# bloomberg/blazingmq

Measured on AMD Instinct MI355X. Metric: device-resident CRC32C GiB/s over batched payloads, 1/2/4/8 MI355X, higher is better.
Workload: dtype u32; 1 GPU; 64k_x_64KiB: 65,536 msgs x 64 KiB per GPU (configs[2], HBM-bound headline); payload_bytes_total=4294967296, seg_bytes=auto, whole_messages=False, parallelism=dp1 (sharded batch, no collective)

## Files before the change

blazingmq_amd/csrc/bmqcrc_host.cpp:

```cpp
#include <hip/hip_runtime.h>
#include <stdint.h>
#include <stdio.h>
#include <stdlib.h>
#include <string.h>

#include <algorithm>
#include <atomic>
#include <condition_variable>
#include <initializer_list>
#include <map>
#include <memory>
#include <mutex>
#include <string>
#include <thread>
#include <utility>
#include <vector>

#include "../../include/bmqcrc.h"
#include "../../include/bmqcrc_protocol.h"
#include "bmqcrc_internal.h"

namespace bmqcrc {
uint32_t cpu_crc32c(const void* data, uint32_t length, uint32_t crc);
uint32_t cpu_combine(uint32_t crcA, uint32_t crcB, uint64_t lenB);
// ... 51 lines not shown
        fresh = true;
        if (p) {
            (void)hipFree(p);
            p = nullptr;
            bytes = 0;
        }
        want = std::max<uint64_t>(want, 256);
        HIP_TRY(hipMalloc(&p, want));
        bytes = want;
        return 0;
    }
    ~DevBuf()
    {
        if (p) {
            (void)hipFree(p);
        }
    }
};

struct PackScratch {
    DevBuf off, first, out, bsum, copy_bsum, ctr;
    uint64_t n = 0;
    bool any = false;
    int ensure(uint64_t n_msgs, int ctr_words, bool need_out)
    {
        int rc;
        if ((rc = ctr.ensure(8 * (ctr_words + kCopyCtrWords))) ||
            (rc = bsum.ensure(8ull * 2 * kPackBlocks)) || (rc = off.ensure(8 * n_msgs))) {
            return rc;
        }
        return need_out ? out.ensure(4 * n_msgs) : 0;
    }
};

struct UnpackScratch {
    DevBuf off, len, exp, out, ctr;
    uint64_t n = 0;
    bool any = false;
    int ensure(uint64_t msg_cap, bool need_out, int ctr_words = kSlotCtrWords)
    {
        const uint64_t slots = std::max<uint64_t>(msg_cap, 1);
        int rc;
        if ((rc = ctr.ensure(8 * ctr_words)) || (rc = off.ensure(8 * slots)) ||
            (rc = len.ensure(4 * slots)) || (rc = exp.ensure(4 * slots))) {
            return rc;
        }
        return need_out ? out.ensure(4 * slots) : 0;
    }
};

struct Workspace {
    std::mutex mu;
    DevBuf seg_first, block_sum, seginfo, firstk, gdesc, grec, bhist, plan_sync;
    uint32_t plan_epoch = 0;
    uint64_t map_wait_ticks = 10000;

    DevBuf arena, offsets, lengths, seeds, out;
    DevBuf expected, vcount, vidx, vblock, buf_crc, first_buf;
    std::vector<std::pair<hipEvent_t, hipEvent_t>> timing, spare;
    uint32_t* hint_host = nullptr;
    uint32_t* hint_dev = nullptr;
    uint32_t last_kernels = 0, last_spec = 0, last_seg = 0, last_map = 0;
    uint32_t last_off_bits = 64, last_off_shift = 0;
    uint32_t void_seen = 0, pair_left = 0;
    DevBuf copy_first, copy_bsum, copy_ctr;
    uint64_t copy_n = 0;
    bool copy_any = false;
    PackScratch pack, rec;
    uint64_t pack_events = 0;
    UnpackScratch unp, runp;
    DevBuf unp_first, unp_bad;
    DevBuf runp_pre, runp_roff, runp_rlen, runp_rflags, runp_bsum;
    UnpackScratch sap;
    DevBuf sap_first, sap_bad, sap_dst, sap_jrn, sap_rec, sap_hdr, sap_pay, sap_meta, sap_bsum;
    DevBuf sap_copy_first, sap_copy_bsum;
    uint32_t sap_lease = 0;
    uint64_t sap_seq = 0;
    UnpackScratch spk;
    DevBuf spk_dst, spk_rec, spk_hdr, spk_type, spk_bsum, spk_copy_first, spk_copy_bsum;
    uint64_t spk_events = 0;
    UnpackScratch ppk;
    DevBuf ppk_dst, ppk_meta, ppk_bsum, ppk_copy_first, ppk_copy_bsum;
    uint64_t ppk_events = 0;
    DevBuf jsel_zero, jsel_rec;
    uint64_t jsel_records = 0;
    bool jsel_any = false;
    uint8_t* pin = nullptr;
    hipEvent_t pin_ev[16] = {};
    bool pin_used[16] = {};
    ~Workspace()
    {
        if (hint_host) {
            (void)hipHostFree(hint_host);
        }
        if (pin) {
            (void)hipHostFree(pin);
        }
        for (hipEvent_t e : pin_ev) {
            if (e) {
                (void)hipEventDestroy(e);
            }
        }
        for (auto& v : {timing, spare}) {
            for (auto& e : v) {
                (void)hipEventDestroy(e.first);
                (void)hipEventDestroy(e.second);
// ... 168 lines not shown
}

struct Ctx {
    int dev = 0;
    DeviceState* st = nullptr;
    hipStream_t s = nullptr;
    Workspace* w = nullptr;
};

int open_ctx(int dev, void* user_stream, Ctx* c)
{
    int rc = device_state(dev, &c->st);
    if (rc) {
        return rc;
    }
    HIP_TRY(hipSetDevice(dev));
    c->dev = dev;
    c->s = (hipStream_t)user_stream;
    c->w = workspace(dev, user_stream);
    return 0;
}

struct LockedCtx : Ctx {
    std::unique_lock<std::mutex> lock;
};

int lock_on(int device, void* stream, bool with_state, LockedCtx* c)
{
    int dev, rc;
    if ((rc = resolve_device(device, &dev))) {
        return rc;
    }
    if (with_state) {
        if ((rc = open_ctx(dev, stream, c))) {
            return rc;
        }
    } else {
        c->dev = dev;
        c->s = (hipStream_t)stream;
        c->w = workspace(dev, stream);
    }
    c->lock = std::unique_lock<std::mutex>(c->w->mu);
    return 0;
}

bool spec_eligible(const Ctx& c, uint64_t n, uint32_t blocks_per_cu)
{
    const uint32_t per_cu = (kTuneBits & 2u) ? 1u : (kTuneBits & 8u) ? 2u : blocks_per_cu;
    const uint64_t waves = (uint64_t)(c.st->num_cus > 0 ? c.st->num_cus : 256) * per_cu *
                           kWavesPerBlock;
    return (n + 63) / 64 >= waves;
}

void auto_shape(uint64_t n, uint64_t arena_bytes, int num_cus, uint32_t* seg,
                uint32_t* blocks_per_cu)
{
    const uint64_t cus = (uint64_t)(num_cus > 0 ? num_cus : 256);
    const uint64_t wave_segs = (uint64_t)kWavesPerBlock * kWaveLanes;
    const bool large = n > 0 && arena_bytes / n >= kDefaultSegBytes;
    if (large && arena_bytes / (4 * kDefaultSegBytes) >= cus * wave_segs) {
        *blocks_per_cu = 1;
        if (*seg == 0) {
            *seg = 4 * kDefaultSegBytes;
        }
        return;
    }
    *blocks_per_cu = 2;
    if (*seg == 0) {
        const uint64_t slots = cus * 2 * wave_segs;
        if (large && arena_bytes / kDefaultSegBytes >= slots) {
            *seg = kDefaultSegBytes;
            return;
        }
        *seg = 256;
        for (uint32_t s : {2048u, 1024u, 512u}) {
            if (arena_bytes / s >= 2 * slots) {
                *seg = s;
                break;
            }
        }
    }
}

uint64_t max_length(const uint32_t* lengths, uint64_t n)
{
    uint32_t m = 0;
    for (uint64_t i = 0; i < n; ++i) {
        m = std::max(m, lengths[i]);
    }
    return m;
}

uint64_t min_length(const uint32_t* lengths, uint64_t n)
{
    uint32_t m = n ? UINT32_MAX : 0u;
    for (uint64_t i = 0; i < n; ++i) {
        m = std::min(m, lengths[i]);
    }
    return m;
}

int run_batch(Ctx& c, uint32_t flags, uint32_t seg, const void* arena, uint64_t arena_bytes,
              const uint64_t* offsets, const uint32_t* lengths, const uint32_t* seeds,
              uint32_t* out, uint64_t n, uint64_t host_max_len = UINT64_MAX,
              uint64_t host_min_len = 0, uint32_t off_shift = 0)
{
    Workspace* w = c.w;
    BatchArgs a;
    memset(&a, 0, sizeof(a));
    a.n = n;
    a.off32 = (flags & BMQCRC_F_OFFSETS32) ? 1u : 0u;
    a.off_shift = a.off32 ? off_shift : 0u;
    auto_shape(n, arena_bytes, c.st->num_cus, &seg, &a.blocks_per_cu);
    a.seg_bytes = seg;
    a.tune = kTuneBits;
    int rc;
    if (flags & BMQCRC_F_WHOLE_MESSAGES) {
        a.whole = 1;
        a.max_segs = n;
    } else if ((rc = plan_ws(w, c.s, n, arena_bytes, seg, &a, *c.st, a.off32 != 0))) {
        return rc;
    } else if (!(kTuneBits & 16u) && !(flags & BMQCRC_F_PLAN)) {
        const uint32_t hint = __atomic_load_n(w->hint_host, __ATOMIC_RELAXED);
        const uint32_t shape = hint & 0xffu, hint_u = hint >> 8;
        if (shape == kHintClosed || shape == kHintIdentity) {
            a.map_planned = 0;
        }
        if (shape == kHintIdentity && spec_eligible(c, n, a.blocks_per_cu)) {
            a.spec = 1;
        } else if (shape == kHintClosed && hint_u >= 2u && hint_u <= 64u && 64u % hint_u == 0u &&
                   (uint64_t)n * hint_u <= 0xFFFFFF00ull) {
            a.spec = hint_u;
        }
    }
    hipStreamCaptureStatus cap = hipStreamCaptureStatusNone;
    const bool capturing = hipStreamIsCapturing(c.s, &cap) == hipSuccess &&
                           cap == hipStreamCaptureStatusActive;
    if (!(kTuneBits & (16u | 4096u)) && !capturing && !a.whole && !a.spec && a.map_planned &&
        w->hint_host &&
        (__atomic_load_n(w->hint_host, __ATOMIC_RELAXED) & 0xffu) != kHintRagged &&
        !(host_max_len != UINT64_MAX && host_max_len > a.seg_bytes &&
          (host_min_len == 0 || (host_min_len - 1) / a.seg_bytes != (host_max_len - 1) / a.seg_bytes))) {
        a.map_planned = 0;
    }
    if ((kTuneBits & 2048u) && !a.whole && (flags & BMQCRC_F_PLAN) &&
        spec_eligible(c, n, a.blocks_per_cu)) {
        a.spec = 1;
    } else if (!a.whole && host_max_len <= a.seg_bytes && !(flags & BMQCRC_F_PLAN)) {
        a.spec = 1;
    } else if (!a.whole && host_min_len > 0 && host_max_len != UINT64_MAX &&
               !(flags & BMQCRC_F_PLAN)) {
        const uint64_t u = (host_max_len - 1) / a.seg_bytes + 1;
        if ((host_min_len - 1) / a.seg_bytes + 1 == u && u >= 2 && u <= 64 && 64 % u == 0 &&
            (uint64_t)n * u <= 0xFFFFFF00ull) {
            a.spec = (uint32_t)u;
        }
    }
    if (!a.whole && !a.spec && a.map_planned && w->hint_host && w->map_wait_ticks != 0) {
        const uint32_t voided = __atomic_load_n(w->hint_host + 1, __ATOMIC_RELAXED);
        if (voided != w->void_seen) {
            w->void_seen = voided;
            w->pair_left = kPairAfterVoid;
        }
        if (w->pair_left) {
            a.pair = 1;
            --w->pair_left;
        }
    }
    if (!a.whole && !a.spec && a.map_planned) {
        if (capturing) {
            a.plan_epoch = 0;
        }
    }
    a.arena = (const uint8_t*)arena;
    a.offsets = offsets;
    a.lengths = lengths;
    a.seeds = seeds;
    a.out = out;
    void* ev0 = nullptr;
    void* ev1 = nullptr;
    if (flags & BMQCRC_F_TIME_KERNEL) {
        std::pair<hipEvent_t, hipEvent_t> ev;
        if (!w->spare.empty()) {
            ev = w->spare.back();
            w->spare.pop_back();
        } else {
            HIP_TRY(hipEventCreate(&ev.first));
            HIP_TRY(hipEventCreate(&ev.second));
        }
        w->timing.push_back(ev);
        ev0 = (void*)ev.first;
        ev1 = (void*)ev.second;
    }
    if (bmqcrc_launch_batch(&a, (void*)c.s, c.st->num_cus, ev0, ev1) != 0) {
        return fail(BMQCRC_EIO, std::string("kernel launch failed: ") +
                                    hipGetErrorString(hipGetLastError()));
    }
    w->last_spec = a.whole ? 1u : a.spec;
    w->last_seg = a.seg_bytes;
    w->last_kernels = n == 0                 ? 0u
                      : (a.whole || a.spec)  ? 1u
                      : !a.map_planned       ? 2u
                      : single_pass_planner(a) ? 2u
                                             : 3u;
    w->last_map = n != 0 && !a.whole && !a.spec && a.map_planned ? 1u : 0u;
    w->last_off_bits = a.off32 ? 32u : 64u;
    w->last_off_shift = a.off_shift;
    return 0;
// ... 2944 lines not shown
```

blazingmq_amd/csrc/bmqcrc_internal.h:

```cpp
#pragma once
#include <stddef.h>
#include <stdint.h>

namespace bmqcrc {

constexpr int kLine = 128;
constexpr int kWaveLanes = 64;
constexpr int kWavesPerBlock = 4;
constexpr int kSlots = 2;
constexpr int kSlotBytes = kWaveLanes * kLine;
constexpr int kLdsBytes = kWavesPerBlock * kSlots * kSlotBytes;
constexpr int kTabBytes = 8 * 256 * 4;
constexpr int kXbBytes = 4 * 256 * 4;
constexpr uint32_t kDefaultSegBytes = 16384;
constexpr int kPlanBlock = 1024;
constexpr int kPlanMaxBlocks = 256;
constexpr int kSyncFlags = 16;

constexpr int kBuckets = 16;

#ifndef BMQCRC_TUNE_BITS
#define BMQCRC_TUNE_BITS 0u
#endif
constexpr uint32_t kTuneBits = BMQCRC_TUNE_BITS;
constexpr uint32_t kRightAlignLines = 1u;

struct BatchArgs {
    const uint8_t* arena;
    const uint64_t* offsets;
    const uint32_t* lengths;
    const uint32_t* seeds;
    uint32_t* out;
    uint32_t* seg_first;
    uint32_t* block_sum;
    uint32_t* seginfo;
    uint32_t* firstk;
    unsigned long long* gdesc;
    uint32_t* grec;
    uint32_t* bhist;
    uint64_t n;
    uint64_t max_segs;
    uint64_t per_msg;
    uint32_t seg_bytes;
    uint32_t nblocks;
    uint32_t whole;
    uint32_t blocks_per_cu;
    uint32_t tune;
    uint32_t map_planned;
    uint32_t* shape_hint;
    uint32_t spec;
    unsigned long long* plan_sync;
    uint32_t plan_epoch;
    uint32_t off32;
    uint64_t map_wait_ticks;
    uint32_t class_desc;
    uint32_t pair;
    uint32_t spread;
    uint32_t off_shift;
};

static_assert(sizeof(BatchArgs) == 200 && offsetof(BatchArgs, plan_epoch) == 168 &&
                  offsetof(BatchArgs, off32) == 172 && offsetof(BatchArgs, map_wait_ticks) == 176 &&
                  offsetof(BatchArgs, spread) == 192 && offsetof(BatchArgs, off_shift) == 196,
              "BatchArgs: kernel argument offsets are fixed");

constexpr uint32_t kPairAfterVoid = 16;

constexpr uint64_t kClassDescGroupsPerWave = 24;

constexpr uint32_t kPlanV = 4;
constexpr uint32_t kSegLast = 0x80000000u;

inline bool single_pass_planner(const BatchArgs& a)
{
    return !(a.tune & 128u) && !a.pair;
}

constexpr uint32_t kHintUnknown = 0;
constexpr uint32_t kHintClosed = 1;
constexpr uint32_t kHintRagged = 2;
constexpr uint32_t kHintIdentity = 3;

constexpr int kCopyWaves = 4;
constexpr uint32_t kCopyChunkPieces = 4096;
constexpr uint32_t kCopyChunkBytes = 16 * kCopyChunkPieces;
constexpr int kCopyPlanThreads = 1024;
constexpr uint32_t kCopyPlanBlocks = 256;
constexpr int kCopyCtrRefused = 0;
constexpr int kCopyCtrLowestInv = 1;
constexpr int kCopyCtrOverflow = 2;
constexpr int kCopyCtrWords = 4;

// ... 439 lines not shown
```

blazingmq_amd/csrc/crc32c_kernels.hip:

```cpp
#include <hip/hip_runtime.h>
#include <stdint.h>

#include <algorithm>

#include "bmqcrc_internal.h"
#include "crc32c_consts.h"
#include "crc32c_diag.h"

namespace bmqcrc {

typedef __attribute__((address_space(3))) uint8_t lds_u8;
typedef __attribute__((address_space(3))) uint32_t lds_u32;
typedef uint32_t u32x4 __attribute__((ext_vector_type(4)));
typedef __attribute__((address_space(3))) const u32x4 lds_cu4;
typedef __attribute__((address_space(3))) u32x4 lds_u4;
typedef uint64_t u64x2 __attribute__((ext_vector_type(2)));
typedef uint32_t u32x4e __attribute__((ext_vector_type(4), aligned(4)));
typedef uint64_t u64x2e __attribute__((ext_vector_type(2), aligned(8)));

__constant__ uint32_t c_x2col[31][32] = BMQCRC_X2COL;
__constant__ uint32_t c_xneg8[136] = BMQCRC_XNEG8;
__constant__ uint32_t c_xbytes[4][256] = BMQCRC_XBYTES;
__constant__ uint32_t c_ty[8][256] = BMQCRC_TY;
__constant__ uint32_t c_rtab11[6144] = BMQCRC_RTAB11;
// ... 714 lines not shown
    const uint32_t lane = (uint32_t)(threadIdx.x & 63);
    const uint32_t key = valid ? r.msg : 0xffffffffu;
    const uint32_t prev = (uint32_t)__shfl_up((int)key, 1);
    const bool head = lane == 0 || prev != key || (key & kSegLast);
    const uint64_t heads = __ballot(head);
    const uint64_t upto = lane == 63 ? ~0ull : ((2ull << lane) - 1ull);
    const uint32_t h = 63u - (uint32_t)__builtin_clzll(heads & upto);
    SegRef o;
    o.msg = key & ~kSegLast;
    o.k = (key & kSegLast) ? kKFromLength : (h == 0 ? r.k : 0u) + (lane - h);
    return o;
}

template <bool O32>
__device__ __forceinline__ uint64_t raw_offset(const BatchArgs& a, uint64_t i)
{
    if constexpr (O32) {
        return ((const uint32_t*)a.offsets)[i];
    } else {
        return a.offsets[i];
    }
}

template <bool O32>
__device__ __forceinline__ uint64_t wide_offset(const BatchArgs& a, uint64_t raw)
{
    if constexpr (O32) {
        return raw << a.off_shift;
    } else {
        return raw;
    }
}

template <bool O32>
__device__ __forceinline__ uint64_t msg_offset(const BatchArgs& a, uint64_t i)
{
    return wide_offset<O32>(a, raw_offset<O32>(a, i));
}

template <bool O32>
__device__ __forceinline__ SegDesc fetch_desc(const BatchArgs& a, SegRef r, bool valid)
{
    SegDesc d = {0ull, r.msg, r.k, 0u, 0u};
    if (valid) {
        d.off = raw_offset<O32>(a, r.msg);
        d.len = a.lengths[r.msg];
        d.seed = a.seeds ? a.seeds[r.msg] : 0u;
    }
    return d;
}

constexpr uint32_t kLongListCap = 64;

template <bool NT, bool ONE, int WPB, bool O32>
__global__ __launch_bounds__(WPB * 64, WPB == 4 ? 2 : 1) void k_fold(BatchArgs a)
{
    constexpr uint32_t kThreads = WPB * 64;
    constexpr int kLds = WPB * kSlots * kSlotBytes;
    constexpr bool H11 = WPB == 8;
    constexpr int kTab = H11 ? (int)kTab11Bytes : kTabBytes;
    __shared__ __attribute__((aligned(16))) uint8_t lds[kTab + kLds + (ONE ? 0 : kXbBytes)];
    __shared__ uint32_t claim_ctr, long_n;
    [[maybe_unused]] __shared__ unsigned long long claim2;
    __shared__ uint32_t long_list[kLongListCap];
    __shared__ uint32_t one_prog[WPB];

    const int lane = threadIdx.x & 63;
    const uint32_t wave = __builtin_amdgcn_readfirstlane(threadIdx.x >> 6);
    const uint32_t tab_lds = (uint32_t)(uintptr_t)(lds_u8*)lds;
    const uint32_t wave_lds = tab_lds + kTab + wave * (kSlots * kSlotBytes);
    const uint32_t xb_lds = tab_lds + kTab + kLds;
    auto remainder = [&](const uint32_t (&Rm)[32], bool skip) -> uint32_t {
        if constexpr (H11) {
            return skip ? tail_bytes8<true>(Rm, tab_lds) : tail_bytes8<false>(Rm, tab_lds);
        } else {
            return skip ? tail_bytes8<true, true>(Rm, tab_lds) : tail_bytes8<false, true>(Rm, tab_lds);
        }
    };
    if (threadIdx.x < (uint32_t)WPB) {
        one_prog[threadIdx.x] = 0u;
    }
    if (threadIdx.x == 0) {
        claim_ctr = WPB;
        claim2 = 0ull;
        long_n = 0;
    }

    constexpr int kTw = (kTab / 4) / (int)kThreads, kXw = 1024 / kThreads;
    static_assert(kTw * (int)kThreads * 4 == kTab && kXw * kThreads == 1024, "table fill");
    constexpr bool kEarly = ONE && WPB == 4;
    static_assert(!kEarly || kTab % (1024 * WPB) == 0, "early tables: whole KiB per wave");
    constexpr bool kNoVgprTab = kEarly;
    const uint32_t gfirst = a.spread ? wave * gridDim.x + blockIdx.x : blockIdx.x * WPB + wave;
    const uint32_t sid = gfirst * 64u + (uint32_t)lane;
    const SegDesc spec = fetch_desc<O32>(a, SegRef{sid, 0u}, sid < a.n);
    uint32_t tw[kNoVgprTab ? 1 : kTw];
#pragma unroll
    for (int i = 0; i < (kNoVgprTab ? 0 : kTw); ++i) {
        const uint32_t t = threadIdx.x + (uint32_t)i * kThreads;
        if constexpr (H11) {
            tw[i] = c_rtab11[t];
        } else {
            tw[i] = c_ty[t >> 8][t & 255u];
        }
    }
    uint32_t xw[kXw];
    if (!ONE) {
#pragma unroll
        for (int i = 0; i < kXw; ++i) {
            const uint32_t t = threadIdx.x + (uint32_t)i * kThreads;
            xw[i] = c_xbytes[t >> 8][t & 255u];
        }
    }
    const uint32_t whole = ONE ? 0u : a.whole;
    const uint32_t spec_mode = ONE ? 1u : a.spec;
    const uint32_t spec_u = spec_mode ? spec_mode : 1u;
    PlanWords pw = {0u, 0u, 0u, 0u};
    uint32_t map_void = 0u;
    uint32_t ep = a.plan_epoch;
    if (!whole && !spec_mode) {
        pw = plan_load(a);
        if (a.map_planned && a.plan_sync) {
            ep = launch_epoch(a);
            map_void = (uint32_t)a.plan_sync[2] == ep;
        }
    }
    __shared__ __attribute__((aligned(16))) uint32_t xneg8[136];
    const uint32_t xn = (!kNoVgprTab && threadIdx.x < 136u) ? c_xneg8[threadIdx.x] : 0u;
    [[maybe_unused]] const uint32_t g0 = blockIdx.x * WPB + wave;
    FOLD_STAMP(0)
#pragma unroll
    for (int i = 0; i < (kNoVgprTab ? 0 : kTw); ++i) {
        const uint32_t t = threadIdx.x + (uint32_t)i * kThreads;
        *(lds_u32*)(uintptr_t)(tab_lds + 4u * t) = tw[i];
    }
    if (!kNoVgprTab && threadIdx.x < 136u) {
        xneg8[threadIdx.x] = xn;
    }
    auto early_tables = [&]() {
        if constexpr (kEarly) {
            constexpr int kKib = kTab / 1024 / WPB;
            const uint64_t src = H11 ? (uint64_t)(uintptr_t)&c_rtab11[0]
                                     : (uint64_t)(uintptr_t)&c_ty[0][0];
            dma_copy_kib<kKib>(tab_lds + 1024u * kKib * wave, src + 1024u * kKib * wave);
            if (wave == 0 && lane < 34) {
                dma_copy_kib<1>((uint32_t)(uintptr_t)xneg8, (uint64_t)(uintptr_t)&c_xneg8[0]);
            }
        }
    };
    auto early_barrier = [&](bool wait) {
        if constexpr (kEarly) {
            if (wait) {
                asm volatile("s_waitcnt vmcnt(0)" ::: "memory");
            }
            __builtin_amdgcn_s_barrier();
        }
    };
    if (!ONE) {
#pragma unroll
        for (int i = 0; i < kXw; ++i) {
            const uint32_t t = threadIdx.x + (uint32_t)i * kThreads;
            *(lds_u32*)(uintptr_t)(xb_lds + 4u * t) = xw[i];
        }
    }

    __shared__ PlanLds pl;
    PlanTotals pt = {(uint32_t)a.n * spec_u, spec_u == 1u ? 1u : 0u, spec_u == 1u ? 0u : spec_u,
                     0u};
    if (!whole && !spec_mode) {
        pt = plan_reduce(a, &pl, pw);
    } else {
        __syncthreads();
    }
    const uint32_t wholef = whole | pt.overflow;
    const uint32_t hint_identity = pt.identity && !pt.overflow;
    const uint32_t hint_uni = pt.uni;
    if (pt.overflow) {
        pt.identity = 1u;
        pt.uni = 0u;
        pt.total = (uint32_t)a.n;
    }
    const uint32_t total = pt.total;
    const uint32_t identity = pt.identity;
    const uint32_t uni = pt.uni;
    const uint32_t sorted =
        (wholef || !a.map_planned || identity || uni || total > a.max_segs || map_void) ? 0u : 1u;
    const uint32_t ngroups = (total + 63u) / 64u;
    const uint32_t SEG = a.seg_bytes;
    const uint64_t arena = (uint64_t)(uintptr_t)a.arena;
    if (a.shape_hint && blockIdx.x == 0 && threadIdx.x == 0 && !whole && !spec_mode) {
        __hip_atomic_store(a.shape_hint,
                           hint_identity ? kHintIdentity
                           : (hint_uni && !pt.overflow && 64u % hint_uni == 0u)
                               ? (kHintClosed | (hint_uni << 8))
                           : (hint_uni || pt.overflow) ? kHintClosed
                                                  : kHintRagged,
                           __ATOMIC_RELAXED, __HIP_MEMORY_SCOPE_SYSTEM);
        if (map_void) {
            __hip_atomic_store(a.shape_hint + 1, ep, __ATOMIC_RELAXED,
                               __HIP_MEMORY_SCOPE_SYSTEM);
        }
    }

    FOLD_STAMP(1)
    const uint32_t rd_off = (uint32_t)lane * 128u + (((uint32_t)lane >> 1) & 7u) * 16u;
    const uint64_t zero = (uint64_t)(uintptr_t)g_zero_line + 16u * ((uint32_t)lane & 7u);

    const uint32_t nbk = gridDim.x;
    auto gid = [&](uint32_t k) {
        if (a.spread) {
            return k * nbk + blockIdx.x;
        }
        const uint32_t r = k / (uint32_t)WPB;
        const uint32_t b = (!ONE && (r & 1u)) ? nbk - 1u - blockIdx.x : blockIdx.x;
        return (b + nbk * r) * (uint32_t)WPB + k % (uint32_t)WPB;
    };
    auto claim_issue = [&]() {
        unsigned long long k = 0;
        if (lane == 0) {
            k = atomicAdd(&claim_ctr, 1u);
        }
        return k;
    };
    auto claim_take = [&](unsigned long long k) {
        return gid((uint32_t)__builtin_amdgcn_readfirstlane((int)(uint32_t)k));
    };
    auto claim = [&]() { return claim_take(claim_issue()); };
    const uint32_t seg_shift = (SEG & (SEG - 1u)) == 0 ? (uint32_t)__builtin_ctz(SEG) : 0u;

    struct Group {
        uint64_t pbase[8];
        uint32_t plo[8], pcnt[8];
        uint64_t E, L0, mend;
        uint32_t msg, k, nseg, nl, R, r0, sl, jE, eE, c0, hskip;
        bool valid, first, lo_part, hi_part;
        bool whole_lines;
    };
    auto setup_lane = [&](bool valid, uint32_t msg, uint32_t k, uint32_t nseg, uint64_t off,
                          uint32_t len, uint32_t seed, Group& G) {
        G.valid = valid;
        G.msg = msg;
        G.k = k;
        G.nseg = valid ? nseg : 0u;
        const uint64_t mstart = arena + off;
        G.mend = mstart + len;
        const SegGeom geo = seg_geom(mstart, len, G.k, G.nseg, SEG);
        G.E = geo.E;
        G.L0 = geo.L0;
        G.first = G.valid && G.k == 0;
        G.nl = G.valid ? geo.nl : 0u;
        G.R = max(wave_max(G.nl), 1u);
        G.hskip = 0u;
        if (G.R == 1u) {
            const uint32_t sl0 = G.valid ? (uint32_t)(geo.S - geo.L0) : 128u;
            G.hskip = __ballot(sl0 < 64u) == 0 ? 8u : 0u;
        }
        G.r0 = G.R - G.nl;
        G.sl = G.valid ? (uint32_t)(geo.S - G.L0) : 0u;
        const uint64_t el = G.valid ? G.E - G.L0 : 0u;
        G.lo_part = (G.sl & 15u) != 0;
        G.hi_part = (el & 15u) != 0;
        G.jE = (uint32_t)(el >> 7);
        G.eE = (uint32_t)(el & 127u);
        G.c0 = ~seed;
        G.whole_lines = __ballot(G.valid && (((geo.S | geo.E) & 127u) != 0)) == 0;
        const uint32_t gS = G.sl >> 4;
        const uint32_t gE = (uint32_t)((el + 15u) >> 4);
        const uint32_t plo_l = 8u * G.r0 + gS;
        const uint32_t pcnt_l = G.valid ? gE - gS : 0u;
        const uint64_t pb_l = G.L0 - ((uint64_t)G.r0 << 7);
        const uint32_t ls = (uint32_t)lane;
        const uint32_t kq = ls >> 3;
        *(lds_u4*)(uintptr_t)(wave_lds + 16u * ((ls & 7u) * 8u + (kq ^ (ls & 7u)))) =
            u32x4{(uint32_t)pb_l, (uint32_t)(pb_l >> 32), plo_l, pcnt_l};
        __builtin_amdgcn_wave_barrier();
#pragma unroll
        for (int i = 0; i < 8; ++i) {
            const u32x4 v = *(lds_cu4*)(uintptr_t)(wave_lds + 16u * (kq * 8u + ((uint32_t)i ^ kq)));
            const uint32_t pp = ((uint32_t)lane & 7u) ^ ((4u * i + ((uint32_t)lane >> 4)) & 7u);
            G.pbase[i] = (((uint64_t)v.y << 32) | v.x) + 16u * pp;
            G.plo[i] = v.z - pp;
            G.pcnt[i] = v.w;
        }
    };
    auto segments = [&](uint32_t len) {
        return len ? (seg_shift ? ((len - 1u) >> seg_shift) : (len - 1u) / SEG) + 1u : 0u;
    };
    bool long_seen = false;
    auto setup = [&](const SegDesc& d, uint32_t gg, Group& G) {
        const uint32_t seg = gg * 64u + (uint32_t)lane;
        bool valid = seg < total;
        uint32_t nseg = !valid ? 0u : (wholef ? 1u : segments(d.len));
        if (spec_mode) {
            const bool ok = spec_u == 1u ? nseg <= 1u : nseg == spec_u;
            if constexpr (ONE) {
                long_seen |= __ballot(valid && !ok) != 0;
            } else if (__ballot(valid && !ok) != 0 && lane == 0) {
                const uint32_t at = atomicAdd(&long_n, 1u);
                if (at < kLongListCap) {
                    long_list[at] = gg;
                }
            }
            valid = valid && ok;
            nseg = spec_u;
        }
        if (ONE) {
            setup_lane(valid, d.msg, 0u, 1u, wide_offset<O32>(a, d.off), d.len, d.seed, G);
        } else {
            setup_lane(valid, d.msg, d.k == kKFromLength ? nseg - 1u : d.k, nseg,
                       wide_offset<O32>(a, d.off), d.len, d.seed, G);
        }
    };
    auto issue_first_rounds = [&](const Group& G) {
        if (!NT || (G.R <= 2u && !G.whole_lines)) {
            dma_round<false>(wave_lds, G.pbase, G.plo, G.pcnt, zero, 0);
            if (G.R > 1) {
                dma_round<false>(wave_lds + kSlotBytes, G.pbase, G.plo, G.pcnt, zero, 1);
            }
            return;
        }
        dma_round<true>(wave_lds, G.pbase, G.plo, G.pcnt, zero, 0);
        if (G.R > 1) {
            dma_round<true>(wave_lds + kSlotBytes, G.pbase, G.plo, G.pcnt, zero, 1);
        }
    };

    auto fold_rounds = [&](const Group& G, uint32_t (&Rm)[32]) {
        uint32_t q[32], p[32];
        const uint32_t R = G.R;
        auto load_line = [&](uint32_t r, uint32_t slot, uint32_t (&m)[32]) {
            const uint32_t j = r - G.r0;
            const bool fx_lo = G.lo_part && j == 0u;
            const bool fx_hi = G.hi_part && j == G.jE;
            const bool fx_sd = G.first && (j == 0u || (j == 1u && G.sl > 124u));
            if (__ballot(fx_lo || fx_hi || fx_sd)) {
                if (fx_lo || fx_hi || fx_sd) {
                    line_fixup(slot, rd_off, fx_lo, G.sl, fx_hi, G.eE, fx_sd,
                               (int)(G.sl - 128u * j), G.c0);
                }
            }
#pragma unroll
            for (int kk = 0; kk < 8; ++kk) {
                const u32x4 v = *(lds_cu4*)(uintptr_t)(slot + (rd_off ^ (16u * kk)));
                m[4 * kk + 0] = v.x;
                m[4 * kk + 1] = v.y;
                m[4 * kk + 2] = v.z;
                m[4 * kk + 3] = v.w;
            }
        };
        for (uint32_t r = 0; r + 1 < R; ++r) {
// ... 1 lines not shown
            asm volatile("s_waitcnt vmcnt(0)" ::: "memory");
            uint32_t m[32];
            load_line(r, slot, m);
            if (r + 2 < R) {
                dma_round<NT>(slot, G.pbase, G.plo, G.pcnt, zero, r + 2);
            }
            if (r == 0) {
                first_round(q, p, m);
            } else {
                fold_round(q, p, m);
            }
        }
        const uint32_t slot = wave_lds + ((R - 1u) & 1u) * kSlotBytes;
        if (R == 1) {
            asm volatile("s_waitcnt vmcnt(0)" ::: "memory");
            load_line(0u, slot, Rm);
            return;
        }
        uint32_t H[32];
        tail_taps(q, p, H);
        asm volatile("s_waitcnt vmcnt(0)" ::: "memory");
        uint32_t m[32];
        load_line(R - 1u, slot, m);
#pragma unroll
        for (int d = 0; d < 32; ++d) {
            Rm[d] = m[d] ^ H[d];
        }
    };

    auto contribution = [&](const Group& C, uint32_t crc) {
        uint32_t contrib = 0;
        const uint32_t padE = C.valid ? (uint32_t)(C.L0 + ((uint64_t)C.nl << 7) - C.E) : 0u;
        if (__ballot(padE != 0) == 0) {
            contrib = C.valid ? crc : 0u;
        } else if (C.valid) {
            contrib = gmul(crc, xneg8[padE]);
        }
        if (ONE) {
            contrib = mul_xpow(contrib, C.valid ? mersenne31(8ull * (C.mend - C.E)) : 0u);
        } else {
            contrib = mul_xbytes(contrib, C.valid ? (uint32_t)(C.mend - C.E) : 0u, xb_lds);
        }
        if (C.first) {
            contrib ^= 0xffffffffu;
        }
        return contrib;
    };
    struct Pending {
        uint32_t msg, val, mode;
    };
    auto commit = [&](const Pending& P) {
        if (P.mode == 1u) {
            a.out[P.msg] = P.val;
        } else if (P.mode == 2u) {
            atomicXor(&a.out[P.msg], P.val);
        }
    };
    auto finish = [&](const Group& C, uint32_t crc) -> Pending {
        Pending P = {C.msg, 0u, 0u};
        if (ONE) {
            uint32_t contrib = C.valid ? crc : 0u;
            const uint32_t padE = C.valid ? (uint32_t)(C.L0 + ((uint64_t)C.nl << 7) - C.E) : 0u;
            if (__ballot(padE != 0) != 0 && C.valid) {
                contrib = gmul(crc, xneg8[padE]);
            }
            P.val = contrib ^ 0xffffffffu;
            P.mode = C.valid ? 1u : 0u;
            return P;
        }
        uint32_t contrib = contribution(C, crc);
        if (__ballot(C.valid && C.nseg != 1u) == 0) {
            P.val = contrib;
            P.mode = C.valid ? 1u : 0u;
            return P;
        }
        const uint32_t key = C.valid ? C.msg : 0xffffffffu;
        const uint32_t pkey = (uint32_t)__shfl_up((int)key, 1);
        const bool head = lane == 0 || pkey != key;
        const uint64_t heads = __ballot(head);
        const uint64_t upto = (lane == 63) ? ~0ull : ((2ull << lane) - 1ull);
        const uint64_t later = heads & ~upto;
        const uint32_t rend = later ? (uint32_t)__builtin_ctzll(later) : 64u;
#pragma unroll
        for (int o = 1; o < 64; o <<= 1) {
            const uint32_t ov = (uint32_t)__shfl_down((int)contrib, o);
            if ((uint32_t)lane + (uint32_t)o < rend) {
                contrib ^= ov;
            }
        }
        P.val = contrib;
        if (C.valid && head) {
            P.mode = (C.k == 0 && rend - (uint32_t)lane == C.nseg) ? 1u : 2u;
        }
        return P;
    };

    auto second_pass = [&](uint32_t nlong) {
        bool any = false;
        const uint32_t mpg = 64u / spec_u;
        const bool listed = nlong <= kLongListCap;
        for (uint32_t j = wave;; j += WPB) {
            const uint32_t gg = ONE ? gfirst + (j / (uint32_t)WPB) * nbk * (uint32_t)WPB
                                : listed ? (j < nlong ? long_list[j] : ngroups) : gid(j);
            if (gg >= ngroups) {
                break;
            }
            const uint64_t i = (uint64_t)gg * mpg + (uint32_t)lane;
            const bool mine = (uint32_t)lane < mpg && i < a.n;
            const uint32_t len = mine ? a.lengths[i] : 0u;
            const uint32_t ns = segments(len);
            uint64_t todo = __ballot(mine && (spec_u == 1u ? ns > 1u : ns != spec_u));
            any = any || todo != 0;
            for (; todo; todo &= todo - 1ull) {
                const uint32_t msg = (uint32_t)((uint64_t)gg * mpg + __builtin_ctzll(todo));
                const uint64_t off = msg_offset<O32>(a, msg);
                const uint32_t mlen = a.lengths[msg];
                const uint32_t seed = a.seeds ? a.seeds[msg] : 0u;
                const uint32_t nseg = segments(mlen);
                uint32_t acc = mlen ? 0u : seed;
                for (uint32_t c = 0; 64u * c < nseg; ++c) {
                    const uint32_t k = 64u * c + (uint32_t)lane;
                    Group H;
                    setup_lane(k < nseg, msg, k, nseg, off, mlen, seed, H);
                    issue_first_rounds(H);
                    uint32_t Rm[32];
                    fold_rounds(H, Rm);
                    uint32_t x = contribution(H, remainder(Rm, false));
#pragma unroll
                    for (int o = 32; o > 0; o >>= 1) {
                        x ^= (uint32_t)__shfl_xor((int)x, o);
                    }
                    acc ^= x;
                }
                if (lane == 0) {
                    a.out[msg] = acc;
                }
            }
        }
        if (any && lane == 0 && a.shape_hint) {
            __hip_atomic_store(a.shape_hint, kHintRagged, __ATOMIC_RELAXED,
                               __HIP_MEMORY_SCOPE_SYSTEM);
        }
    };

    Group G;
    SegDesc nxt = {0ull, 0u, 0u, 0u, 0u};
    SegRef ref2 = {0u, 0u};
    if constexpr (ONE) {
        const uint32_t stride = nbk * (uint32_t)WPB;
        uint32_t g = gfirst;
        if (g < ngroups) {
            const uint32_t s0 = g * 64u + (uint32_t)lane;
            SegRef r0 = {0u, 0u};
            if (!identity) {
                r0 = map_segment(a, &pl, s0, s0 < total, identity, uni, sorted, ep);
                if (sorted) {
                    r0 = resolve_sorted(r0, s0 < total);
                }
            }
            const SegDesc d0 = identity ? spec : fetch_desc<O32>(a, r0, s0 < total);
            const uint32_t s1 = (g + stride) * 64u + (uint32_t)lane;
            const bool v1 = g + stride < ngroups && s1 < total;
            SegRef r1 = map_segment(a, &pl, s1, v1, identity, uni, sorted, ep);
            if (sorted) {
                r1 = resolve_sorted(r1, v1);
            }
            if constexpr (!kNoVgprTab) {
// ... 33 lines not shown
                        __builtin_amdgcn_s_setprio(1);
                    }
                    ++it;
                }
            }
            uint32_t Rm[32];
            fold_rounds(G, Rm);
            if (meet) {
                early_barrier(false);
                meet = false;
            }
            if (first) {
                FOLD_STAMP(3)
                first = false;
            }
            if (g + stride >= ngroups) {
                FOLD_STAMP(4)
            }
            const Group C = G;
            if (g + stride < ngroups) {
                setup(nxt, g + stride, G);
                const uint32_t s2 = (g + 2u * stride) * 64u + (uint32_t)lane;
                const bool v2 = g + 2u * stride < ngroups && s2 < total;
                nxt = fetch_desc<O32>(a, sorted ? resolve_sorted(ref2, v2) : ref2, v2);
                const uint32_t s3 = (g + 3u * stride) * 64u + (uint32_t)lane;
                ref2 = map_segment(a, &pl, s3, g + 3u * stride < ngroups && s3 < total, identity,
                                   uni, sorted, ep);
                issue_first_rounds(G);
            }
            commit(pend);
            pend = finish(C, remainder(Rm, C.hskip != 0u));
        }
        commit(pend);
    } else {
    uint32_t g = gid(wave), g1 = ngroups, g2 = ngroups;
    if (g < ngroups) {
        g1 = claim();
        g2 = g1 < ngroups ? claim() : ngroups;
        const uint32_t s0 = g * 64u + (uint32_t)lane;
        SegRef r0 = {0u, 0u};
        if (!identity) {
            r0 = map_segment(a, &pl, s0, s0 < total, identity, uni, sorted, ep);
            if (sorted) {
                r0 = resolve_sorted(r0, s0 < total);
            }
        }
        const SegDesc d0 = identity ? spec : fetch_desc<O32>(a, r0, s0 < total);
        const uint32_t s1 = g1 * 64u + (uint32_t)lane;
        const bool v1 = g1 < ngroups && s1 < total;
        SegRef r1 = map_segment(a, &pl, s1, v1, identity, uni, sorted, ep);
        if (sorted) {
            r1 = resolve_sorted(r1, v1);
        }
        nxt = fetch_desc<O32>(a, r1, v1);
        const uint32_t s2 = g2 * 64u + (uint32_t)lane;
        ref2 = map_segment(a, &pl, s2, g2 < ngroups && s2 < total, identity, uni, sorted, ep);
        setup(d0, g, G);
        issue_first_rounds(G);
        FOLD_STAMP(2)
    }
    bool first_group = true;
    Pending pend = {0u, 0u, 0u};
    while (g < ngroups) {
        const bool more = g1 < ngroups && g2 < ngroups;
        const unsigned long long k3 = more ? claim_issue() : 0ull;
        uint32_t Rm[32];
        fold_rounds(G, Rm);
        if (first_group) {
            FOLD_STAMP(3)
            first_group = false;
        }
        if (g1 >= ngroups) {
            FOLD_STAMP(4)
        }
        const Group C = G;
        uint32_t g3 = ngroups;
        if (g1 < ngroups) {
            setup(nxt, g1, G);
            const uint32_t s2 = g2 * 64u + (uint32_t)lane;
            const bool v2 = g2 < ngroups && s2 < total;
            nxt = fetch_desc<O32>(a, sorted ? resolve_sorted(ref2, v2) : ref2, v2);
            g3 = more ? claim_take(k3) : ngroups;
            const uint32_t s3 = g3 * 64u + (uint32_t)lane;
            ref2 = map_segment(a, &pl, s3, g3 < ngroups && s3 < total, identity, uni, sorted, ep);
            issue_first_rounds(G);
        }
        commit(pend);
        pend = finish(C, remainder(Rm, C.hskip != 0u));
        g = g1;
        g1 = g2;
        g2 = g3;
    }
    commit(pend);
    }
    FOLD_STAMP(5)
    if constexpr (ONE) {
        if (long_seen) {
            second_pass(0u);
        }
    } else if (spec_mode) {
        __syncthreads();
        const uint32_t nlong = long_n;
        if (nlong) {
            second_pass(nlong);
        }
    }
    FOLD_STAMP(6)
}

__device__ __forceinline__ uint32_t size_class(uint32_t nl)
{
    nl |= 1u;
    const uint32_t b = 31u - __clz(nl);
    const uint32_t c = b ? 2u * b + ((nl >> (b - 1u)) & 1u) : 0u;
    return c < kBuckets - 1 ? c : kBuckets - 1;
}

__device__ __forceinline__ uint32_t msg_segments(const BatchArgs& a, uint64_t off, uint32_t len,
                                                 uint32_t seg_shift, uint32_t* c_last)
{
// ... 544 lines not shown

}

using namespace bmqcrc;

template <bool O32>
static int launch_batch(const BatchArgs* a, void* stream, int num_cus, void* ev_start,
                        void* ev_stop)
{
    hipStream_t s = (hipStream_t)stream;
    if (a->n == 0) {
        return 0;
    }
    if (!a->whole && !a->spec && a->map_planned && a->plan_epoch == 0) {
        hipLaunchKernelGGL(k_epoch_advance, dim3(1), dim3(1), 0, s, a->plan_sync);
    }
    if (!a->whole && !a->spec) {
        const bool single_pass = single_pass_planner(*a);
        if (a->map_planned && single_pass) {
            hipLaunchKernelGGL(O32 ? k_plan_map32 : k_plan_map, dim3(a->nblocks), dim3(kPlanBlock), 0, s, *a);
        } else if (a->map_planned) {
            hipLaunchKernelGGL((k_plan<true, O32>), dim3(a->nblocks), dim3(kPlanBlock), 0, s, *a);
        } else {
            hipLaunchKernelGGL((k_plan<false, O32>), dim3(a->nblocks), dim3(kPlanBlock), 0, s, *a);
        }
        if (a->map_planned && !single_pass) {
            hipLaunchKernelGGL(k_plan_sort<O32>, dim3(a->nblocks), dim3(kPlanBlock), 0, s, *a);
        }
    }
    const uint64_t max_groups = (a->max_segs + 63) / 64;
    const uint32_t per_cu = (a->tune & 2u) ? 1u : (a->tune & 8u) ? 2u : a->blocks_per_cu;
    const uint64_t cus = (uint64_t)(num_cus > 0 ? num_cus : 256);
    const bool wide = per_cu == 2u && !(a->tune & 1024u) && max_groups >= 2u * 8u * cus;
    const uint32_t wpb = wide ? 8u : 4u;
    uint64_t grid = (max_groups + wpb - 1) / wpb;
    const uint64_t cap = wide ? cus : cus * (per_cu ? per_cu : 2u);
    if (grid > cap) {
        grid = cap;
    }
    if (grid < 1) {
        grid = 1;
    }
    if (ev_start) {
        (void)hipEventRecord((hipEvent_t)ev_start, s);
    }
    const bool one = a->spec == 1u && !a->whole && !(a->tune & 64u);
    BatchArgs b = *a;
    b.spread = 0u;
    if (!wide && grid < cus && max_groups > grid) {
        grid = std::min<uint64_t>(max_groups, cus);
        b.spread = 1u;
    }
    const dim3 gd((unsigned)grid), bd(wpb * 64u);
    if (a->tune & 1u) {
        if (wide) {
            hipLaunchKernelGGL((k_fold<false, false, 8, O32>), gd, bd, 0, s, b);
        } else {
            hipLaunchKernelGGL((k_fold<false, false, 4, O32>), gd, bd, 0, s, b);
        }
    } else if (one) {
        if (wide) {
            hipLaunchKernelGGL((k_fold<true, true, 8, O32>), gd, bd, 0, s, b);
        } else {
            hipLaunchKernelGGL((k_fold<true, true, 4, O32>), gd, bd, 0, s, b);
        }
    } else if (wide) {
        hipLaunchKernelGGL((k_fold<true, false, 8, O32>), gd, bd, 0, s, b);
    } else {
        hipLaunchKernelGGL((k_fold<true, false, 4, O32>), gd, bd, 0, s, b);
    }
    if (ev_stop) {
        (void)hipEventRecord((hipEvent_t)ev_stop, s);
    }
    return hipGetLastError() == hipSuccess ? 0 : -5;
}

extern "C" int bmqcrc_launch_batch(const BatchArgs* a, void* stream, int num_cus, void* ev_start,
                                   void* ev_stop)
{
    return a->off32 ? launch_batch<true>(a, stream, num_cus, ev_start, ev_stop)
                    : launch_batch<false>(a, stream, num_cus, ev_start, ev_stop);
}

extern "C" int bmqcrc_plan_map_occupancy(int off32, int* blocks_per_cu)
{
    int per = 0;
    const void* k = off32 ? reinterpret_cast<const void*>(&k_plan_map32)
                          : reinterpret_cast<const void*>(&k_plan_map);
    if (hipOccupancyMaxActiveBlocksPerMultiprocessor(&per, k, kPlanBlock, 0) != hipSuccess) {
        return -5;
    }
    *blocks_per_cu = per;
    return 0;
}

extern "C" int bmqcrc_launch_compare(const uint32_t* got, const uint32_t* expected, uint64_t n,
                                     uint32_t* bad_count, uint32_t* bad_idx, uint32_t bad_cap,
                                     void* stream)
{
    if (n == 0) {
        return 0;
    }
    const uint64_t blocks = std::min<uint64_t>((n + 255) / 256, 4096);
    hipLaunchKernelGGL(k_compare, dim3((unsigned)blocks), dim3(256), 0, (hipStream_t)stream, got,
                       expected, n, bad_count, bad_idx, bad_cap);
    return hipGetLastError() == hipSuccess ? 0 : -5;
}
// ... 51 lines not shown
```

Measured before the change: 6590 GiB/s.

## Add SPEC kernel variant for uniform multi-group messages with arrival counters

```diff
diff --git a/blazingmq_amd/csrc/bmqcrc_host.cpp b/blazingmq_amd/csrc/bmqcrc_host.cpp
--- a/blazingmq_amd/csrc/bmqcrc_host.cpp
+++ b/blazingmq_amd/csrc/bmqcrc_host.cpp
@@ -127,6 +127,8 @@
 struct Workspace {
     std::mutex mu;
     DevBuf seg_first, block_sum, seginfo, firstk, gdesc, grec, bhist, plan_sync;
+    DevBuf arrive;
+    bool arrive_zeroed = false;
     uint32_t plan_epoch = 0;
     uint64_t map_wait_ticks = 10000;
 
@@ -401,6 +403,12 @@
     return (n + 63) / 64 >= waves;
 }
 
+bool spec_uniform(uint64_t u, uint64_t n)
+{
+    return u >= 2 && (u <= 64 ? 64 % u == 0 : u % 64 == 0 && u < (1u << 24)) &&
+           n * u <= 0xFFFFFF00ull;
+}
+
 void auto_shape(uint64_t n, uint64_t arena_bytes, int num_cus, uint32_t* seg,
                 uint32_t* blocks_per_cu)
 {
@@ -477,8 +485,7 @@
         }
         if (shape == kHintIdentity && spec_eligible(c, n, a.blocks_per_cu)) {
             a.spec = 1;
-        } else if (shape == kHintClosed && hint_u >= 2u && hint_u <= 64u && 64u % hint_u == 0u &&
-                   (uint64_t)n * hint_u <= 0xFFFFFF00ull) {
+        } else if (shape == kHintClosed && spec_uniform(hint_u, n)) {
             a.spec = hint_u;
         }
     }
@@ -500,9 +507,23 @@
     } else if (!a.whole && host_min_len > 0 && host_max_len != UINT64_MAX &&
                !(flags & BMQCRC_F_PLAN)) {
         const uint64_t u = (host_max_len - 1) / a.seg_bytes + 1;
-        if ((host_min_len - 1) / a.seg_bytes + 1 == u && u >= 2 && u <= 64 && 64 % u == 0 &&
-            (uint64_t)n * u <= 0xFFFFFF00ull) {
+        if ((host_min_len - 1) / a.seg_bytes + 1 == u && spec_uniform(u, n)) {
             a.spec = (uint32_t)u;
+        }
+    }
+    if (a.spec > 64u) {
+        if ((rc = w->arrive.ensure(8 * n))) {
+            return rc;
+        }
+        w->arrive_zeroed = w->arrive_zeroed && !w->arrive.fresh;
+        if (!w->arrive_zeroed && capturing) {
+            a.spec = 0;
+        } else if (!w->arrive_zeroed) {
+            HIP_TRY(hipMemsetAsync(w->arrive.p, 0, w->arrive.bytes, c.s));
+            w->arrive_zeroed = true;
+        }
+        if (a.spec) {
+            a.arrive = (unsigned long long*)w->arrive.p;
         }
     }
     if (!a.whole && !a.spec && a.map_planned && w->hint_host && w->map_wait_ticks != 0) {
diff --git a/blazingmq_amd/csrc/bmqcrc_internal.h b/blazingmq_amd/csrc/bmqcrc_internal.h
--- a/blazingmq_amd/csrc/bmqcrc_internal.h
+++ b/blazingmq_amd/csrc/bmqcrc_internal.h
@@ -37,7 +37,10 @@
     uint32_t* firstk;
     unsigned long long* gdesc;
     uint32_t* grec;
-    uint32_t* bhist;
+    union {
+        uint32_t* bhist;
+        unsigned long long* arrive;
+    };
     uint64_t n;
     uint64_t max_segs;
     uint64_t per_msg;
diff --git a/blazingmq_amd/csrc/crc32c_kernels.hip b/blazingmq_amd/csrc/crc32c_kernels.hip
--- a/blazingmq_amd/csrc/crc32c_kernels.hip
+++ b/blazingmq_amd/csrc/crc32c_kernels.hip
@@ -790,9 +790,10 @@
 
 constexpr uint32_t kLongListCap = 64;
 
-template <bool NT, bool ONE, int WPB, bool O32>
+template <bool NT, bool ONE, int WPB, bool O32, bool SPEC = false>
 __global__ __launch_bounds__(WPB * 64, WPB == 4 ? 2 : 1) void k_fold(BatchArgs a)
 {
+    static_assert(!(ONE && SPEC), "ONE is a speculative kernel of its own");
     constexpr uint32_t kThreads = WPB * 64;
     constexpr int kLds = WPB * kSlots * kSlotBytes;
     constexpr bool H11 = WPB == 8;
@@ -826,7 +827,7 @@
 
     constexpr int kTw = (kTab / 4) / (int)kThreads, kXw = 1024 / kThreads;
     static_assert(kTw * (int)kThreads * 4 == kTab && kXw * kThreads == 1024, "table fill");
-    constexpr bool kEarly = ONE && WPB == 4;
+    constexpr bool kEarly = (ONE || SPEC) && WPB == 4;
     static_assert(!kEarly || kTab % (1024 * WPB) == 0, "early tables: whole KiB per wave");
     constexpr bool kNoVgprTab = kEarly;
     const uint32_t gfirst = a.spread ? wave * gridDim.x + blockIdx.x : blockIdx.x * WPB + wave;
@@ -843,7 +844,7 @@
         }
     }
     uint32_t xw[kXw];
-    if (!ONE) {
+    if (!ONE && !kEarly) {
 #pragma unroll
         for (int i = 0; i < kXw; ++i) {
             const uint32_t t = threadIdx.x + (uint32_t)i * kThreads;
@@ -853,10 +854,12 @@
     const uint32_t whole = ONE ? 0u : a.whole;
     const uint32_t spec_mode = ONE ? 1u : a.spec;
     const uint32_t spec_u = spec_mode ? spec_mode : 1u;
+    const uint32_t gpm = (SPEC && spec_u > 64u) ? spec_u / 64u : 1u;
+    const bool planned = !SPEC && !whole && !spec_mode;
     PlanWords pw = {0u, 0u, 0u, 0u};
     uint32_t map_void = 0u;
     uint32_t ep = a.plan_epoch;
-    if (!whole && !spec_mode) {
+    if (planned) {
         pw = plan_load(a);
         if (a.map_planned && a.plan_sync) {
             ep = launch_epoch(a);
@@ -881,6 +884,11 @@
             const uint64_t src = H11 ? (uint64_t)(uintptr_t)&c_rtab11[0]
                                      : (uint64_t)(uintptr_t)&c_ty[0][0];
             dma_copy_kib<kKib>(tab_lds + 1024u * kKib * wave, src + 1024u * kKib * wave);
+            if constexpr (!ONE) {
+                static_assert(kXbBytes == 1024 * WPB, "early tables: a KiB of move factors per wave");
+                dma_copy_kib<1>(xb_lds + 1024u * wave,
+                                (uint64_t)(uintptr_t)&c_xbytes[0][0] + 1024u * wave);
+            }
             if (wave == 0 && lane < 34) {
                 dma_copy_kib<1>((uint32_t)(uintptr_t)xneg8, (uint64_t)(uintptr_t)&c_xneg8[0]);
             }
@@ -894,7 +902,7 @@
             __builtin_amdgcn_s_barrier();
         }
     };
-    if (!ONE) {
+    if (!ONE && !kEarly) {
 #pragma unroll
         for (int i = 0; i < kXw; ++i) {
             const uint32_t t = threadIdx.x + (uint32_t)i * kThreads;
@@ -905,7 +913,7 @@
     __shared__ PlanLds pl;
     PlanTotals pt = {(uint32_t)a.n * spec_u, spec_u == 1u ? 1u : 0u, spec_u == 1u ? 0u : spec_u,
                      0u};
-    if (!whole && !spec_mode) {
+    if (planned) {
         pt = plan_reduce(a, &pl, pw);
     } else {
         __syncthreads();
@@ -926,10 +934,12 @@
     const uint32_t ngroups = (total + 63u) / 64u;
     const uint32_t SEG = a.seg_bytes;
     const uint64_t arena = (uint64_t)(uintptr_t)a.arena;
-    if (a.shape_hint && blockIdx.x == 0 && threadIdx.x == 0 && !whole && !spec_mode) {
+    if (a.shape_hint && blockIdx.x == 0 && threadIdx.x == 0 && planned) {
         __hip_atomic_store(a.shape_hint,
                            hint_identity ? kHintIdentity
-                           : (hint_uni && !pt.overflow && 64u % hint_uni == 0u)
+                           : (hint_uni && !pt.overflow &&
+                              (64u % hint_uni == 0u ||
+                               (hint_uni % 64u == 0u && hint_uni < (1u << 24))))
                                ? (kHintClosed | (hint_uni << 8))
                            : (hint_uni || pt.overflow) ? kHintClosed
                                                   : kHintRagged,
@@ -1033,7 +1043,7 @@
             const bool ok = spec_u == 1u ? nseg <= 1u : nseg == spec_u;
             if constexpr (ONE) {
                 long_seen |= __ballot(valid && !ok) != 0;
-            } else if (__ballot(valid && !ok) != 0 && lane == 0) {
+            } else if (__ballot(valid && !ok) != 0 && lane == 0 && gg % gpm == 0u) {
                 const uint32_t at = atomicAdd(&long_n, 1u);
                 if (at < kLongListCap) {
                     long_list[at] = gg;
@@ -1141,8 +1151,18 @@
     auto commit = [&](const Pending& P) {
         if (P.mode == 1u) {
             a.out[P.msg] = P.val;
-        } else if (P.mode == 2u) {
+        } else if (!SPEC && P.mode == 2u) {
             atomicXor(&a.out[P.msg], P.val);
+        } else if (SPEC && P.mode == 3u) {
+            unsigned long long* const word = a.arrive + P.msg;
+            __hip_atomic_fetch_xor(word, (unsigned long long)P.val, __ATOMIC_RELAXED,
+                                   __HIP_MEMORY_SCOPE_AGENT);
+            const unsigned long long before = __hip_atomic_fetch_add(
+                word, 1ull << 32, __ATOMIC_RELAXED, __HIP_MEMORY_SCOPE_AGENT);
+            if ((uint32_t)(before >> 32) + 1u == gpm) {
+                __hip_atomic_store(word, 0ull, __ATOMIC_RELAXED, __HIP_MEMORY_SCOPE_AGENT);
+                a.out[P.msg] = (uint32_t)before;
+            }
         }
     };
     auto finish = [&](const Group& C, uint32_t crc) -> Pending {
@@ -1179,14 +1199,14 @@
         }
         P.val = contrib;
         if (C.valid && head) {
-            P.mode = (C.k == 0 && rend - (uint32_t)lane == C.nseg) ? 1u : 2u;
+            P.mode = (C.k == 0 && rend - (uint32_t)lane == C.nseg) ? 1u : SPEC ? 3u : 2u;
         }
         return P;
     };
 
     auto second_pass = [&](uint32_t nlong) {
         bool any = false;
-        const uint32_t mpg = 64u / spec_u;
+        const uint32_t mpg = gpm > 1u ? 1u : 64u / spec_u;
         const bool listed = nlong <= kLongListCap;
         for (uint32_t j = wave;; j += WPB) {
             const uint32_t gg = ONE ? gfirst + (j / (uint32_t)WPB) * nbk * (uint32_t)WPB
@@ -1194,14 +1214,15 @@
             if (gg >= ngroups) {
                 break;
             }
-            const uint64_t i = (uint64_t)gg * mpg + (uint32_t)lane;
-            const bool mine = (uint32_t)lane < mpg && i < a.n;
+            const uint64_t m0 = (uint64_t)(gg / gpm) * mpg;
+            const uint64_t i = m0 + (uint32_t)lane;
+            const bool mine = (uint32_t)lane < mpg && i < a.n && gg % gpm == 0u;
             const uint32_t len = mine ? a.lengths[i] : 0u;
             const uint32_t ns = segments(len);
             uint64_t todo = __ballot(mine && (spec_u == 1u ? ns > 1u : ns != spec_u));
             any = any || todo != 0;
             for (; todo; todo &= todo - 1ull) {
-                const uint32_t msg = (uint32_t)((uint64_t)gg * mpg + __builtin_ctzll(todo));
+                const uint32_t msg = (uint32_t)(m0 + __builtin_ctzll(todo));
                 const uint64_t off = msg_offset<O32>(a, msg);
                 const uint32_t mlen = a.lengths[msg];
                 const uint32_t seed = a.seeds ? a.seeds[msg] : 0u;
@@ -1341,20 +1362,37 @@
         if (sorted) {
             r1 = resolve_sorted(r1, v1);
         }
-        nxt = fetch_desc<O32>(a, r1, v1);
+        if constexpr (!kEarly) {
+            nxt = fetch_desc<O32>(a, r1, v1);
+        }
         const uint32_t s2 = g2 * 64u + (uint32_t)lane;
         ref2 = map_segment(a, &pl, s2, g2 < ngroups && s2 < total, identity, uni, sorted, ep);
         setup(d0, g, G);
+        if constexpr (kEarly) {
+            __builtin_amdgcn_s_waitcnt(0x0F70);
+        }
         issue_first_rounds(G);
+        early_tables();
+        if constexpr (kEarly) {
+            nxt = fetch_desc<O32>(a, r1, v1);
+        }
         FOLD_STAMP(2)
+    } else {
+        early_tables();
+        early_barrier(true);
     }
     bool first_group = true;
+    bool meet = kEarly;
     Pending pend = {0u, 0u, 0u};
     while (g < ngroups) {
         const bool more = g1 < ngroups && g2 < ngroups;
         const unsigned long long k3 = more ? claim_issue() : 0ull;
         uint32_t Rm[32];
         fold_rounds(G, Rm);
+        if (meet) {
+            early_barrier(false);
+            meet = false;
+        }
         if (first_group) {
             FOLD_STAMP(3)
             first_group = false;
@@ -2005,7 +2043,20 @@
         b.spread = 1u;
     }
     const dim3 gd((unsigned)grid), bd(wpb * 64u);
-    if (a->tune & 1u) {
+    const bool closed = a->whole || a->spec >= 2u;
+    if (closed && (a->tune & 1u)) {
+        if (wide) {
+            hipLaunchKernelGGL((k_fold<false, false, 8, O32, true>), gd, bd, 0, s, b);
+        } else {
+            hipLaunchKernelGGL((k_fold<false, false, 4, O32, true>), gd, bd, 0, s, b);
+        }
+    } else if (closed) {
+        if (wide) {
+            hipLaunchKernelGGL((k_fold<true, false, 8, O32, true>), gd, bd, 0, s, b);
+        } else {
+            hipLaunchKernelGGL((k_fold<true, false, 4, O32, true>), gd, bd, 0, s, b);
+        }
+    } else if (a->tune & 1u) {
         if (wide) {
             hipLaunchKernelGGL((k_fold<false, false, 8, O32>), gd, bd, 0, s, b);
         } else {
```

Result: no change. 6585 GiB/s, median of 2 (-0.1%).
